# ZhenlongYuan/TSAR-MVS

Hardware: AMD Instinct MI355X
Metric: depthmap Mpixels/sec (ETH3D full-res, 8 iters) (higher is better)
Workload: dtype f32

## Files before the change

### include/tsar.h

```cpp
#ifndef TSAR_H_
#define TSAR_H_

#include <stddef.h>
#include <stdint.h>

#ifdef __cplusplus
extern "C" {
#endif

#define TSAR_MAX_VIEWS 64
#define TSAR_MAXCOST 2.0f

#define TSAR_OK 0
#define TSAR_ERR_INVALID (-1)
#define TSAR_ERR_HIP (-2)
#define TSAR_ERR_STATE (-3)
#define TSAR_ERR_NOMEM (-4)

#define TSAR_MEM_HOST 0
#define TSAR_MEM_DEVICE 1

#define TSAR_COMB_ALL 0
#define TSAR_COMB_BEST_N 1
#define TSAR_COMB_ANGLE 2
// ... 159 lines not shown
void* tsar_device_alloc(int device, size_t bytes);
void tsar_device_free(int device, void* p);
int tsar_device_write(int device, void* dst, const void* host_src, size_t bytes);
int tsar_peer_copy(int dst_device, void* dst, int src_device, const void* src, size_t bytes);

int tsar_enable_kernel_timing(tsar_ctx* ctx, int enable);
int tsar_reset_kernel_timing(tsar_ctx* ctx);
int tsar_get_kernel_timing(tsar_ctx* ctx, tsar_kernel_timing* out, int cap, int* n_out);

int tsar_selftest_sqrt(tsar_ctx* ctx, int mode, uint64_t seed, uint64_t* mismatches_out);
int tsar_selftest_divide(tsar_ctx* ctx, const float* X, const float* Y, const float* Z, size_t n, float* u_out, float* v_out, int ieee);
int tsar_selftest_divide_random(tsar_ctx* ctx, int log2_triples, uint64_t seed, int mode, int guarded, uint64_t* mismatches_out,
                                uint64_t* outside_guard_out);
int tsar_selftest_sweep_census(tsar_ctx* ctx, int colour, uint64_t* out8);
int tsar_selftest_sweep_repeat(tsar_ctx* ctx, int colour, void* memo_dev, uint64_t* out8);
int tsar_selftest_slic_stage(tsar_ctx* ctx, int stage, int w, int h, int mw, int mh, const tsar_slic_settings* s, const void* in0,
                             const void* in1, void* inout);

#ifdef __cplusplus
}
#endif
#endif
```

### tsar-mvs_amd/api.py

```python
from __future__ import annotations

import ctypes as C
import os

import numpy as np

_HERE = os.path.dirname(os.path.abspath(__file__))
LIB_PATH = os.environ.get("TSAR_LIB") or os.path.join(_HERE, "libtsar_hip.so")

TSAR_OK = 0
TSAR_ERR_INVALID, TSAR_ERR_HIP, TSAR_ERR_STATE, TSAR_ERR_NOMEM = -1, -2, -3, -4
MEM_HOST, MEM_DEVICE = 0, 1
COMB_ALL, COMB_BEST_N, COMB_ANGLE, COMB_GOOD = 0, 1, 2, 3
FLAG_FIX_DOWN_FAR_SEED, FLAG_FIX_RIGHT_FAR_CMP, FLAG_STRICT_DIV = 1, 2, 4
FLAG_FIX_PLANE_FIT = 8
FLAG_NO_LINE_CLOSING = 16
FLAG_TEX_FILTER_8BIT = 32
FLAG_FIX_INIT_RADIUS = 64
MAXCOST = 2.0
MAX_VIEWS = 64


class TsarError(RuntimeError):
    def __init__(self, code, msg):
# ... 42 lines not shown
ABI_SYMBOLS = [
    "tsar_create", "tsar_destroy", "tsar_last_error", "tsar_version", "tsar_get_stream", "tsar_synchronize",
    "tsar_default_params", "tsar_set_params", "tsar_set_views", "tsar_set_views_u8", "tsar_set_view_subset",
    "tsar_pm_init", "tsar_pm_iterate", "tsar_pm_iterate_final", "tsar_pm_sweep", "tsar_set_sweep_counter", "tsar_pm_cost_planes", "tsar_set_plane", "tsar_get_plane",
    "tsar_load_planes", "tsar_compute_disp", "tsar_compute_disp_final", "tsar_depth_to_plane", "tsar_get_result",
    "tsar_pyramid_views", "tsar_upsample_planes", "tsar_compute_disp_final_upsampled", "tsar_get_view_image",
    "tsar_set_geom_depths", "tsar_clear_geom", "tsar_pm_rescore", "tsar_get_geom_matrices",
    "tsar_geom_pyramid", "tsar_pyramid_planes", "tsar_upsample_merge",
    "tsar_default_geom_check_params", "tsar_geom_check",
    "tsar_default_geom_reproject_params", "tsar_geom_reproject", "tsar_pm_merge_depths",
    "tsar_default_plane_prior_params", "tsar_set_plane_prior", "tsar_clear_plane_prior", "tsar_get_plane_prior",
    "tsar_set_reliable_mask", "tsar_get_reliable_mask", "tsar_lrdiff", "tsar_getview", "tsar_wmf", "tsar_set_regions", "tsar_detect_weak_texture", "tsar_ransac_regions",
    "tsar_set_region_planes", "tsar_fake_depth", "tsar_fill_textureless",
    "tsar_default_slic_settings", "tsar_slic", "tsar_default_fusion_params", "tsar_fuse", "tsar_fuse_ctx",
    "tsar_host_alloc", "tsar_host_free", "tsar_device_alloc", "tsar_device_free", "tsar_device_write", "tsar_peer_copy", "tsar_enable_kernel_timing", "tsar_reset_kernel_timing", "tsar_get_kernel_timing",
    "tsar_selftest_divide", "tsar_selftest_divide_random", "tsar_selftest_sqrt", "tsar_selftest_sweep_census", "tsar_selftest_sweep_repeat", "tsar_selftest_slic_stage",
]

_lib = None


def load_library(path: str = LIB_PATH):
    global _lib
    if _lib is not None:
        return _lib
    if not os.path.exists(path):
        raise ImportError(f"{path} not found: build it with `make -C tsar-mvs_amd/csrc` "
                          "(or __graft_entry__.build()); there is no CPU fallback")
    L = C.CDLL(path)
    L.tsar_last_error.restype = C.c_char_p
    L.tsar_last_error.argtypes = [C.c_void_p]
# ... 66 lines not shown
    L.tsar_fake_depth.argtypes = [C.c_void_p, C.c_void_p, C.c_int]
    L.tsar_fill_textureless.argtypes = [C.c_void_p]
    L.tsar_slic.argtypes = [C.c_void_p, C.c_void_p, C.c_int, C.c_int, C.POINTER(SlicSettings), C.c_void_p, C.c_int]
    L.tsar_default_fusion_params.restype = None
    L.tsar_default_fusion_params.argtypes = [C.POINTER(FusionParams)]
    L.tsar_fuse.argtypes = [C.c_int, C.c_int, C.c_int, C.c_int, C.POINTER(Camera), C.POINTER(C.c_void_p), C.POINTER(C.c_void_p), C.POINTER(C.c_void_p), C.c_int,
                            C.c_void_p, C.c_void_p, C.POINTER(FusionParams), C.c_void_p, C.c_int64, C.POINTER(C.c_int64)]
    L.tsar_fuse_ctx.argtypes = [C.c_void_p] + list(L.tsar_fuse.argtypes[1:])
    L.tsar_get_stream.argtypes = [C.c_void_p, C.POINTER(C.c_void_p)]
    L.tsar_synchronize.argtypes = [C.c_void_p]
    L.tsar_enable_kernel_timing.argtypes = [C.c_void_p, C.c_int]
    L.tsar_reset_kernel_timing.argtypes = [C.c_void_p]
    L.tsar_get_kernel_timing.argtypes = [C.c_void_p, C.POINTER(KernelTiming), C.c_int, C.POINTER(C.c_int)]
    L.tsar_selftest_divide.argtypes = [C.c_void_p, C.c_void_p, C.c_void_p, C.c_void_p, C.c_size_t, C.c_void_p, C.c_void_p, C.c_int]
    L.tsar_selftest_sweep_census.argtypes = [C.c_void_p, C.c_int, C.POINTER(C.c_uint64)]
    L.tsar_selftest_sweep_repeat.argtypes = [C.c_void_p, C.c_int, C.c_void_p, C.POINTER(C.c_uint64)]
    L.tsar_selftest_sqrt.argtypes = [C.c_void_p, C.c_int, C.c_uint64, C.POINTER(C.c_uint64)]
    L.tsar_selftest_divide_random.argtypes = [C.c_void_p, C.c_int, C.c_uint64, C.c_int, C.c_int, C.POINTER(C.c_uint64), C.POINTER(C.c_uint64)]
    L.tsar_selftest_slic_stage.argtypes = [C.c_void_p, C.c_int, C.c_int, C.c_int, C.c_int, C.c_int, C.POINTER(SlicSettings), C.c_void_p, C.c_void_p, C.c_void_p]
    _lib = L
    return L


def default_params(**kw) -> Params:
    p = Params()
    load_library().tsar_default_params(C.byref(p))
    for k, v in kw.items():
        setattr(p, k, v)
    return p

# ... 305 lines not shown
        assert X.shape == Y.shape == Z.shape
        u, v = np.empty_like(X), np.empty_like(X)
        self._chk(self.L.tsar_selftest_divide(self._ctx, _ptr(X)[0], _ptr(Y)[0], _ptr(Z)[0], X.size, _ptr(u)[0], _ptr(v)[0], int(ieee) if mode is None else mode))
        return u, v

    def selftest_sqrt(self, mode: int, seed: int = 0) -> int:
        bad = C.c_uint64(0)
        self._chk(self.L.tsar_selftest_sqrt(self._ctx, mode, seed, C.byref(bad)))
        return bad.value

    def selftest_sweep_census(self, colour: int) -> dict:
        out = (C.c_uint64 * 8)()
        self._chk(self.L.tsar_selftest_sweep_census(self._ctx, colour, out))
        keys = ("waves", "arms_any_lane", "max_lane_survivors", "max_lane_survivors_nodup", "lane_survivors", "lane_survivors_nodup", "pixels", "arms_present")
        return dict(zip(keys, [int(v) for v in out]))

    def selftest_divide_random(self, log2_triples: int, seed: int, mode: int, guarded: bool = True):
        bad, out = C.c_uint64(0), C.c_uint64(0)
        self._chk(self.L.tsar_selftest_divide_random(self._ctx, log2_triples, seed, mode, int(guarded), C.byref(bad), C.byref(out)))
        return bad.value, out.value

    def _slic_stage(self, stage, w, h, mw, mh, settings, in0, in1, inout):
        p1 = _ptr(in1)[0] if in1 is not None else None
        self._chk(self.L.tsar_selftest_slic_stage(self._ctx, stage, w, h, mw, mh, C.byref(settings), _ptr(in0)[0], p1, _ptr(inout)[0]))
        return inout

    def slic_convert(self, bgra, color_space=0):
        img = np.ascontiguousarray(bgra, np.uint8).reshape(-1, 4)
        return self._slic_stage(0, img.shape[0], 1, 0, 0, SlicSettings(20, 0, 5.0, 0, color_space), img, None, np.zeros((img.shape[0], 4), np.float32))

# ... 272 lines not shown
```

### tsar-mvs_amd/csrc/pm_core.h

```cpp
#pragma once
#include <type_traits>

#include "tsar_device_math.h"

#define PM_BLOCK 256
#define PM_RW 32

#include "pm_tap_common.h"

template <bool QUAD, bool DIFF = false>
DEVFN float sample_bilinear(const DevView& vw, int w, int h, int qpitch, float u, float v, bool q8 = false) {
    u = fminf(fmaxf(u, -1.0f), (float)w);
    v = fminf(fmaxf(v, -1.0f), (float)h);
    const float fu = floorf(u), fv = floorf(v);
    float ax = u - fu, ay = v - fv;
    if (q8) { ax = rintf(ax * 256.0f) * 0.00390625f; ay = rintf(ay * 256.0f) * 0.00390625f; }
    const int iu = (int)fu, iv = (int)fv;
    float t00, t10, t01, t11;
    if (QUAD) {
        const uint32_t off = (uint32_t)(__mul24(iv + 1, qpitch) + iu + 1) * 4u;
        const uint32_t q = *(global_u32_ptr)((const char __attribute__((address_space(1)))*)vw.quad + off);
        t00 = (float)(q & 0xffu);
        t10 = (float)((q >> 8) & 0xffu);
        t01 = (float)((q >> 16) & 0xffu);
// ... 134 lines not shown
    const prior_entry q = ((const __attribute__((address_space(1))) prior_entry*)pp)[y * sc->w + x];
    const float Dp = q.w;
    const float a = fabsf(D - Dp);
    const float rel = a / Dp;
    const float dclip = sc->prior_depth_clip, nclip = sc->prior_normal_clip;
    const float r_d = rel < dclip ? rel / dclip : 1.0f;
    const float s = 1.0f - ((n4.x * q.x + n4.y * q.y) + n4.z * q.z);
    const float s0 = s < 0.0f ? 0.0f : s;
    const float r_n = s < nclip ? s0 / nclip : 1.0f;
    const float t = (sc->prior_weight_depth * r_d) + (sc->prior_weight_normal * r_n);
    return Dp > 0.0f ? c + t : c;
}

template <int NB, int HR, bool STRICT, bool QUAD, int V = 0, int BLK = PM_BLOCK>
DEVFN float multiview_cost(const DevScene* __restrict__ sc, const typename TileOf<QUAD>::type* tile, int tw, int own, const float* wts, const PixelRef& pr,
                           int x, int y, const float4& n4, int& beview, float& ratio) {
    constexpr bool GEOM = (V & TSAR_V_GEOM) != 0;
    constexpr int VT = V & ~(TSAR_V_GEOM | TSAR_V_REDRAW);
    float best[NB];
#pragma unroll
    for (int k = 0; k < NB; k++) best[k] = __builtin_inff();
    const int num = sc->n_sel;
    int valid = 0, bv = -1;
    float cmin = __builtin_inff();
    float depth_h = 0.0f;
    if constexpr (GEOM) depth_h = plane_depth(sc->ref, n4, x, y);
    int vi_next = sc->sel[0];
    for (int i = 0; i < num; i++) {
        const int vi = vi_next;
        vi_next = sc->sel[i + 1 < num ? i + 1 : i];
        float c;
        if constexpr ((VT & TSAR_V_LUT) != 0) c = view_cost_lut<STRICT, (VT >> 11) & 7, (VT & TSAR_V_BUF) != 0 && !STRICT, (VT & TSAR_V_MIX) != 0 && !STRICT>(sc, sc->view[vi], tile, tw, own, wts, pr, x, y, n4);
        else if constexpr (QUAD && HR == 5 && r5_production_variant(VT))
            c = view_cost_r5<STRICT, (VT & 128) != 0 && !STRICT, (VT & 8) != 0, (VT & TSAR_V_BUF) != 0, (VT & TSAR_V_MIX) != 0, BLK>(sc, sc->view[vi], tile, tw, own, wts, pr, x, y, n4);
#ifdef TSAR_EXPERIMENTS
        else if constexpr (QUAD && HR == 5 && r5_diag_variant(VT))
            c = view_cost_r5<false, true, true, true, true, BLK, (VT & 4194304) ? 1 : 2>(sc, sc->view[vi], tile, tw, own, wts, pr, x, y, n4);
#endif
        else {
            static_assert(VT == 0, "unknown tap-loop variant");
            c = view_cost_generic<HR, STRICT, QUAD, BLK>(sc, sc->view[vi], tile, tw, own, wts, pr, x, y, n4);
        }
        auto vmin = [](float a, float b) { float r; asm("v_min_f32 %0, %1, %2" : "=v"(r) : "v"(a), "v"(b)); return r; };
        auto vmax = [](float a, float b) { float r; asm("v_max_f32 %0, %1, %2" : "=v"(r) : "v"(a), "v"(b)); return r; };
        c = vmin(c, TSAR_MAXCOST);
        valid -= (int32_t)__float_as_uint(c - TSAR_MAXCOST) >> 31;
        if constexpr (GEOM) c = c + geom_term(sc, sc->view[vi], vi, x, y, depth_h);
        {
// ... 47 lines not shown
```

### tsar-mvs_amd/csrc/pm_sweep.hip

```cpp
#include "pm_sweep_impl.h"

__global__ void d16_probe_kernel(uint32_t* out) {
    __shared__ unsigned short t[64];
    t[threadIdx.x] = (unsigned short)(0x4300u + threadIdx.x);
    __syncthreads();
    uint32_t r = 0xffffffffu;
    const uint32_t addr = (uint32_t)(uintptr_t)(const __attribute__((address_space(3))) unsigned short*)(t + threadIdx.x);
    asm volatile("ds_read_u16_d16_hi %0, %1\n\ts_waitcnt lgkmcnt(0)" : "+v"(r) : "v"(addr));
    out[threadIdx.x] = r;
}
bool probe_d16_hi_zeroes(tsar_ctx* ctx) {
    CallFrame f(ctx, "d16 probe", nullptr, false);
    uint32_t h[64];
    uint32_t* d = f.out(h, 64, TSAR_MEM_HOST);
    if (f.ok()) {
        hipLaunchKernelGGL(d16_probe_kernel, dim3(1), dim3(64), 0, ctx->stream, d);
        f.launched();
    }
    bool ok = f.finish() == TSAR_OK;
    for (int i = 0; ok && i < 64; i++) ok = h[i] == ((0x4300u + i) << 16);
    return ok;
}

template <int NB, int HR>
static int launch_sweep_nh(tsar_ctx* ctx, int colour, const PlaneBuf& a, const PlaneBuf& b, const PlaneBuf& c, uint32_t sid, int dp, int dr) {
    const bool strict = ctx->hscene.flags & TSAR_FLAG_STRICT_DIV, quad = ctx->hscene.use_quad;
    const bool buf = ctx->buffer_gather && ctx->sweeps_done >= (strict ? (ctx->buffer_from > 2 ? ctx->buffer_from : 2) : ctx->buffer_from);
    const int v = ctx->variant;
    if constexpr ((NB == 2 || NB == 4) && HR == 5)
    if (quad && !(ctx->hscene.flags & TSAR_FLAG_TEX_FILTER_8BIT) && (v == 250 || v == 122 || (v == 114 && NB == 2))) {
#define SWEEP_R5(S, V, B) (buf ? launch_sweep_g<NB, 5, S, true, (V) | TSAR_V_BUF, B>(ctx, colour, a, b, c, sid, dp, dr) : launch_sweep_g<NB, 5, S, true, V, B>(ctx, colour, a, b, c, sid, dp, dr))
        const bool mix = buf && !strict && v == 250 && ctx->hscene.n_sel > 0 && ctx->hscene.view[ctx->hscene.sel[0]].dquad != nullptr;
#define SWEEP_R5_FAST250(B) (mix ? launch_sweep_g<NB, 5, false, true, 250 | TSAR_V_BUF | TSAR_V_MIX, B>(ctx, colour, a, b, c, sid, dp, dr) : SWEEP_R5(false, 250, B))
        if constexpr (NB == 2) {
            const int tiles256 = ((ctx->hscene.w + PM_RW - 1) / PM_RW) * ((ctx->hscene.h + 15) / 16);
            bool small = tiles256 < SWEEP_SMALL_IMAGE_TILES;
            if (ctx->force_block) small = ctx->force_block == 128;
            if (small && v != 114) {
                if (strict) return SWEEP_R5(true, 122, 128);
                return v == 250 ? SWEEP_R5_FAST250(128) : launch_sweep_g<2, 5, false, true, 122, 128>(ctx, colour, a, b, c, sid, dp, dr);
            }
            if (v == 114) return strict ? launch_sweep_g<2, 5, true, true, 114>(ctx, colour, a, b, c, sid, dp, dr) : launch_sweep_g<2, 5, false, true, 114>(ctx, colour, a, b, c, sid, dp, dr);
        }
        if (strict) return SWEEP_R5(true, 122, PM_BLOCK);
        return v == 250 ? SWEEP_R5_FAST250(PM_BLOCK) : launch_sweep_g<NB, 5, false, true, 122>(ctx, colour, a, b, c, sid, dp, dr);
#undef SWEEP_R5_FAST250
#undef SWEEP_R5
    }
    constexpr int NBG = NB == 4 ? 32 : NB;
    if (strict) return quad ? launch_sweep_g<NBG, HR, true, true>(ctx, colour, a, b, c, sid, dp, dr) : launch_sweep_g<NBG, HR, true, false>(ctx, colour, a, b, c, sid, dp, dr);
    return quad ? launch_sweep_g<NBG, HR, false, true>(ctx, colour, a, b, c, sid, dp, dr) : launch_sweep_g<NBG, HR, false, false>(ctx, colour, a, b, c, sid, dp, dr);
}

int launch_pm_sweep(tsar_ctx* ctx, int colour, const PlaneBuf& same_in, const PlaneBuf& other, const PlaneBuf& same_out, uint32_t stream_id,
                    int do_prop, int do_refine) {
    const DevScene& hs = ctx->hscene;
#ifdef TSAR_EXPERIMENTS
    if (!scene_has_terms(hs)) {
        int launched = 0;
        const int rc = launch_pm_sweep_experiment(ctx, colour, same_in, other, same_out, stream_id, do_prop, do_refine, &launched);
        if (rc != TSAR_OK || launched) return rc;
// ... 13 lines not shown
```

### tsar-mvs_amd/csrc/pm_sweep_impl.h

```cpp
#pragma once
#include "pm_dispatch.h"

#define SWEEP_SMALL_IMAGE_TILES 3072

#define CAND_SAME (1 << 30)

DEVFN void select_candidates(const DevScene* __restrict__ sc, const float* __restrict__ c_same, const float* __restrict__ c_other,
                             int x, int y, int cand[8]) {
    const int col = sc->w, row = sc->h;
    const int p = y * col + x;
    const bool fix_seed = sc->flags & TSAR_FLAG_FIX_DOWN_FAR_SEED, fix_cmp = sc->flags & TSAR_FLAG_FIX_RIGHT_FAR_CMP;
    float cmin;
    int cp, cs;
#pragma unroll
    for (int k = 0; k < 8; k++) cand[k] = -1;
    if (y > 2) {
        cp = p - 3 * col; cmin = c_other[cp];
#pragma unroll
        for (int i = 1; i < 11; ++i)
            if (y > 2 + 2 * i) { const int q = p - (3 + 2 * i) * col; const float v = c_other[q]; if (v < cmin) { cmin = v; cp = q; } }
        cand[0] = cp;
    }
    if (y < row - 3) {
        cp = p + 3 * col;
// ... 60 lines not shown
    }
}

DEVFN bool same_bits(const float4& a, const float4& b) {
    return __float_as_uint(a.x) == __float_as_uint(b.x) && __float_as_uint(a.y) == __float_as_uint(b.y) &&
           __float_as_uint(a.z) == __float_as_uint(b.z) && __float_as_uint(a.w) == __float_as_uint(b.w);
}

struct SweepMemo {
    int32_t* cand;
    uint32_t* seq;
    uint32_t* changed;
    uint32_t launch, valid_from;
    int mode;
    int slot_off;
};

template <int NB, int HR, bool STRICT, bool QUAD, int V = 0, int BLK = PM_BLOCK, bool CMP = false>
__global__ __launch_bounds__(BLK) void pm_sweep_kernel(const DevScene* __restrict__ sc, int colour,
                                                            const float* __restrict__ c_same, const float4* __restrict__ n_same,
                                                            const float* __restrict__ c_other, const float4* __restrict__ n_other,
                                                            float* c_out, float4* n_out, float* __restrict__ ratio_out,
                                                            int32_t* __restrict__ beview_out, uint32_t stream_id, int do_prop,
                                                            int do_refine, int tiles_x, int n_tiles, int cost_consistent, int strip_w,
                                                            const float* __restrict__ final_text, SweepMemo memo) {
    extern __shared__ __attribute__((aligned(16))) unsigned char lds_raw[];
    typedef typename TileOf<QUAD>::type TileT;
    constexpr int RW = PM_RW;
    constexpr int SWEEP_RH = 2 * BLK / RW;
    const int hr = HR > 0 ? HR : sc->hrad, vr = HR > 0 ? HR : sc->vrad;
    const int tw = RW + 2 * hr, th = SWEEP_RH + 2 * vr;
// ... 99 lines not shown
                    const float dispOut = fminf(fmaxf(disp + dz, sc->min_disp), sc->max_disp);
                    depth_t = fb / dispOut;
                    float nt[3];
                    nt[0] = n_now.x + between(rn.u[1], -deltaN, deltaN);
                    nt[1] = n_now.y + between(rn.u[2], -deltaN, deltaN);
                    nt[2] = n_now.z + between(rn.u[3], -deltaN, deltaN);
                    const float inv = 1.0f / sqrtf(dot3(nt, nt));
                    nt[0] *= inv; nt[1] *= inv; nt[2] *= inv;
                    if (dot3(nt, vv) > 0.0f) { nt[0] = -nt[0]; nt[1] = -nt[1]; nt[2] = -nt[2]; }
                    n_t.x = nt[0]; n_t.y = nt[1]; n_t.z = nt[2];
                    n_t.w = plane_offset(rf, nt, x, y, depth_t);
                    deltaN = deltaN / 4.0f;
                    deltaZ = deltaZ / 10.0f;
                }
                int bv; float rt;
                const float cost_t = multiview_cost<NB, HR, STRICT, QUAD, V, BLK>(sc, tile, tw, own, wts, pr, x, y, n_t, bv, rt);
                if (cost_t < cost_now) {
                    cost_now = cost_t; n_now = n_t; depth_now = depth_t;
                    ratio_w = rt; beview_w = bv; wrote = true;
                }
            }
        }
    } else {
        const int lane = threadIdx.x & 63, wave0 = threadIdx.x & ~63;
        volatile int32_t* slot_ci = (volatile int32_t*)(lds_raw + memo.slot_off) + wave0;
        volatile unsigned short* slot_src = (volatile unsigned short*)(lds_raw + memo.slot_off + 4 * BLK) + wave0;
        auto pixel_of = [&](int tid, int& px, int& py, int& pown) {
            const int sly = tid >> 4, sk = tid & 15;
            py = ty0 + sly;
            const int slx = 2 * sk + ((colour + py) & 1);
            px = tx0 + slx;
// ... 89 lines not shown
                    depth_t = fb / dispOut;
                    float nt[3];
                    nt[0] = n_now.x + between(rn.u[1], -dN, dN);
                    nt[1] = n_now.y + between(rn.u[2], -dN, dN);
                    nt[2] = n_now.z + between(rn.u[3], -dN, dN);
                    const float inv = 1.0f / sqrtf(dot3(nt, nt));
                    nt[0] *= inv; nt[1] *= inv; nt[2] *= inv;
                    if (dot3(nt, ev) > 0.0f) { nt[0] = -nt[0]; nt[1] = -nt[1]; nt[2] = -nt[2]; }
                    n_t.x = nt[0]; n_t.y = nt[1]; n_t.z = nt[2];
                    n_t.w = plane_offset(rf, nt, ex, ey, depth_t);
                }
            }
            const float* ewts = LUTW ? wts_base : wts_base + etid;
            int bv = -1;
            float rt = 0.f, cost_t = TSAR_MAXCOST;
            if (go) cost_t = multiview_cost<NB, HR, STRICT, QUAD, V, BLK>(sc, tile, tw, eown, ewts, epr, ex, ey, n_t, bv, rt);
            if (it < trips) {
                arms_of_trip(lo, [&](int a, int j, bool has) {
                    const float c = __int_as_float(__builtin_amdgcn_ds_bpermute((j & 63) << 2, __float_as_int(cost_t)));
                    const float r = __int_as_float(__builtin_amdgcn_ds_bpermute((j & 63) << 2, __float_as_int(rt)));
                    const int b = __builtin_amdgcn_ds_bpermute((j & 63) << 2, bv);
                    if (has && c < cost_now) {
                        cost_now = c; acc_arm = a;
                        ratio_w = r; beview_w = b;
                    }
                });
            } else if (go && cost_t < cost_now) {
                cost_now = cost_t; n_now = n_t; depth_now = depth_t;
                ratio_w = rt; beview_w = bv;
            }
        }
// ... 11 lines not shown
            c_out[pp] = cost_now;
            n_out[pp] = n_now;
            if (changed && !final_text) { ratio_out[pp] = ratio_w; beview_out[pp] = beview_w; }
            if (changed && memo.mode) memo.changed[pp] = memo.launch;
            return;
        }
    }
    c_out[p] = cost_now;
    n_out[p] = n_now;
    if (wrote && !final_text) { ratio_out[p] = ratio_w; beview_out[p] = beview_w; }
    if (wrote && memo.mode) memo.changed[p] = memo.launch;
}


template <int HR, bool QUAD, int V>
constexpr bool sweep_has_packed_form() { return QUAD && ((HR == 5 && r5_production_variant(V & ~TSAR_V_GEOM)) || (V & TSAR_V_LUT) != 0); }

template <int NB, int HR, bool STRICT, bool QUAD, int V = 0, int BLK = PM_BLOCK>
static int launch_sweep_t(tsar_ctx* ctx, int colour, const PlaneBuf& same_in, const PlaneBuf& other, const PlaneBuf& same_out,
                          uint32_t stream_id, int do_prop, int do_refine) {
    constexpr int SWEEP_RH = 2 * BLK / PM_RW;
#ifdef TSAR_EXPERIMENTS
    const size_t lds_pad = ctx->lds_pad;
#else
    constexpr size_t lds_pad = 0;
#endif
    SweepMemo memo;
    memo.cand = ctx->memo_cand; memo.seq = ctx->memo_seq; memo.changed = ctx->changed_seq;
    memo.launch = ctx->launch_seq; memo.valid_from = ctx->memo_valid_from;
    memo.mode = (ctx->memo_mode && ctx->memo_cand && ctx->cost_consistent && !ctx->final_text) ? 1 : 0;
    bool packed = false;
    if constexpr (sweep_has_packed_form<HR, QUAD, V>())
        packed = memo.mode && do_prop && ctx->compact_from >= 0 && ctx->call_launch >= ctx->compact_from;
    auto kern = pm_sweep_kernel<NB, HR, STRICT, QUAD, V, BLK, false>;
    if constexpr (sweep_has_packed_form<HR, QUAD, V>())
        if (packed) kern = pm_sweep_kernel<NB, HR, STRICT, QUAD, V, BLK, true>;
    const size_t slots = packed ? 6 * (size_t)BLK : 0;
    TapGrid g;
    if (const int rc = tap_grid(ctx, kern, SWEEP_RH, BLK, QUAD, V, lds_pad + slots, g)) return rc;
    memo.slot_off = packed ? (int)(g.lds - slots) : 0;
    {
        ScopedKernelTimer tm(ctx, (V & TSAR_V_GEOM) ? "pm_sweep_geom" : "pm_sweep");
        ScopedKernelTimer tm_packed(ctx, packed ? "pm_sweep_packed" : nullptr);
        hipLaunchKernelGGL(kern, dim3(g.n_tiles), dim3(BLK), g.lds, ctx->stream, ctx->dscene, colour, same_in.c, same_in.n4, other.c,
                           other.n4, same_out.c, same_out.n4, ctx->ratio, ctx->beview, stream_id, do_prop, do_refine, g.tiles_x, g.n_tiles,
                           ctx->cost_consistent ? 1 : 0, strip_width(ctx->strip_w, g.tiles_x), ctx->final_text, memo);
    }
    TSAR_HIP_TRY(ctx, hipGetLastError());
    return TSAR_OK;
}

template <int NB, int HR, bool STRICT, bool QUAD, int V = 0, int BLK = PM_BLOCK>
static int launch_sweep_g(tsar_ctx* ctx, int colour, const PlaneBuf& same_in, const PlaneBuf& other, const PlaneBuf& same_out,
                          uint32_t stream_id, int do_prop, int do_refine) {
    if (scene_has_terms(ctx->hscene)) return launch_sweep_t<NB, HR, STRICT, QUAD, V | TSAR_V_GEOM, BLK>(ctx, colour, same_in, other, same_out, stream_id, do_prop, do_refine);
    return launch_sweep_t<NB, HR, STRICT, QUAD, V, BLK>(ctx, colour, same_in, other, same_out, stream_id, do_prop, do_refine);
}
```

### tsar-mvs_amd/csrc/pm_tap_common.h

```cpp
#pragma once

typedef const uint32_t __attribute__((address_space(1)))* global_u32_ptr;
typedef const float __attribute__((address_space(1)))* global_f32_ptr;

template <bool STRICT, bool ROW = false>
DEVFN void tap_line_base(const float* H, float a, float& bx, float& by, float& bz) {
    bx = STRICT ? H[0] * a : fma_(H[ROW ? 1 : 0], a, H[2]);
    by = STRICT ? H[3] * a : fma_(H[ROW ? 4 : 3], a, H[5]);
    bz = STRICT ? H[6] * a : fma_(H[ROW ? 7 : 6], a, H[8]);
}
template <bool STRICT, bool ROW = false>
DEVFN void tap_homogeneous(const float* H, float t, float bx, float by, float bz, float& X, float& Y, float& Z) {
    X = fma_(H[ROW ? 0 : 1], t, bx); Y = fma_(H[ROW ? 3 : 4], t, by); Z = fma_(H[ROW ? 6 : 7], t, bz);
    if (STRICT) { X += H[2]; Y += H[5]; Z += H[8]; }
}
DEVFN void pixel_homogeneous(const float* H, float xi, float yj, float& X, float& Y, float& Z) {
    float bx, by, bz;
    tap_line_base<false>(H, xi, bx, by, bz);
    tap_homogeneous<false>(H, yj, bx, by, bz, X, Y, Z);
}

template <bool STRICT, bool GUARD>
DEVFN void tap_divide(float X, float Y, float Z, float& u, float& v) {
    if (STRICT) {
// ... 99 lines not shown
    float mean_ref;
    float var_ref;
    bool textured;
};
DEVFN PixelRef pixel_ref_from_sums(float sum_ref, float sum_ref_ref, float inv_wsum) {
    PixelRef pr;
    pr.inv_wsum = inv_wsum;
    sum_ref *= pr.inv_wsum;
    sum_ref_ref *= pr.inv_wsum;
    pr.mean_ref = sum_ref;
    pr.var_ref = sum_ref_ref - sum_ref * sum_ref;
    pr.textured = !(pr.var_ref < 1e-5f);
    return pr;
}

DEVFN float ncc_cost(const PixelRef& pr, TapSums t) {
    t.src *= pr.inv_wsum;
    t.src_src *= pr.inv_wsum;
    t.ref_src *= pr.inv_wsum;
    const float var_src = t.src_src - t.src * t.src;
    if (var_src < 1e-5f) return TSAR_MAXCOST;
    const float covar = t.ref_src - pr.mean_ref * t.src;
    const float vrs = sqrt_rsq_exact(pr.var_ref * var_src);
    return fmaxf(0.0f, fminf(TSAR_MAXCOST, 1.0f - covar / vrs));
}
```

### tsar-mvs_amd/csrc/pm_tap_r5.h

```cpp
#pragma once

template <bool STRICT, bool ROW, bool D16, bool BUF, bool MIX, int BLK, int DIAG = 0>
DEVFN float view_cost_r5(const DevScene* __restrict__ sc, const DevView& vw, const unsigned short* tile, int tw, int own, const float* wts,
                         const PixelRef& pr, int x, int y, const float4& n4) {
    static_assert(!(STRICT && ROW), "the row-wise walk changes the summation order: fast mode only");
    static_assert(!MIX || (BUF && !STRICT), "the half-float difference texture serves the fast arithmetic's blend through buffer loads");
    const int w = sc->w, h = sc->h, qp = sc->quad_pitch;
    const int qorg = quad_border_bytes(qp);
    float H[9];
    if (STRICT) plane_homography(sc->ref, vw, n4, H, sc->k_sparse != 0);
    else plane_homography_fast(sc->ref, vw, n4, H);
    float sum_src = 0.f, sum_src_src = 0.f, sum_ref_src = 0.f;
    bool need_clamp;
    if (!STRICT) {
        float Xc, Yc, Zc;
        pixel_homogeneous(H, (float)x, (float)y, Xc, Yc, Zc);
        const float a = fabsf(H[0]) + fabsf(H[1]), b = fabsf(H[3]) + fabsf(H[4]), c = fabsf(H[6]) + fabsf(H[7]);
        const float Zmin = fma_(-5.0f, c, Zc);
        const float r = __builtin_amdgcn_rcpf(Zmin * Zc);
        const float r5 = 5.0f * r, rc = Zmin * r;
        const float du = fma_(a, Zc, fabsf(Xc) * c) * r5, dv = fma_(b, Zc, fabsf(Yc) * c) * r5;
        const float uc = Xc * rc, vc = Yc * rc;
        const bool inside = Zmin > 0.0f && fminf(uc - du, vc - dv) >= 1.5f && uc + du <= (float)(w - 1) - 1.5f && vc + dv <= (float)(h - 1) - 1.5f;
        need_clamp = !__all(inside);
// ... 100 lines not shown
            if (MIX) s = blend_dquad(q2[jj], ax[jj], ay[jj]);
            else s = blend_quad<!STRICT>(q[jj], ax[jj], ay[jj]);
            if (jj == 0 && DIAG != 2) {
                if (D16)
                    asm("s_waitcnt lgkmcnt(0)" : "+v"(rcol[0]), "+v"(rcol[1]), "+v"(rcol[2]), "+v"(rcol[3]), "+v"(rcol[4]), "+v"(rcol[5]),
                        "+v"(wcol[0]), "+v"(wcol[1]), "+v"(wcol[2]), "+v"(s));
                else
                    asm("s_waitcnt lgkmcnt(0)" : "+v"(wcol[0]), "+v"(wcol[1]), "+v"(wcol[2]), "+v"(s));
            }
            const float r = D16 ? rcol[jj] : tile_value(ROW ? tile[own + i * tw + (2 * jj - 5)] : tile[own + (2 * jj - 5) * tw + i]);
            const float wt = wcol[jj >> 1][jj & 1];
            const TapSums t = tap_accumulate<STRICT>(TapSums{sum_src, sum_src_src, sum_ref_src}, wt, r, s);
            sum_src = t.src; sum_src_src = t.src_src; sum_ref_src = t.ref_src;
        }
    };
    if (need_clamp) {
#pragma unroll 1
        for (int i = -5; i <= 5; i += 2) line6(i, std::true_type(), std::false_type());
    } else if constexpr (MIX) {
#pragma unroll
        for (int i = -5; i <= 5; i += 2) line6(i, std::false_type(), std::true_type());
    } else {
#pragma unroll 1
        for (int i = -5; i <= 5; i += 2) line6(i, std::false_type(), std::false_type());
    }
    return ncc_cost(pr, TapSums{sum_src, sum_src_src, sum_ref_src});
}

__host__ __device__ constexpr bool r5_diag_variant(int V) { return V == (250 | TSAR_V_BUF | TSAR_V_MIX | 4194304) || V == (250 | TSAR_V_BUF | TSAR_V_MIX | 8388608); }
__host__ __device__ constexpr bool r5_production_variant(int V) { return V == 114 || V == 122 || V == 250 || V == (114 | TSAR_V_BUF) || V == (122 | TSAR_V_BUF) || V == (250 | TSAR_V_BUF) || V == (250 | TSAR_V_BUF | TSAR_V_MIX); }
```

### tsar-mvs_amd/csrc/tsar_api.hip

```cpp
#include <math.h>
#include <stdio.h>
#include <stdlib.h>
#include <string.h>

#include <algorithm>

#include "tsar_dev.h"

ScopedKernelTimer::ScopedKernelTimer(tsar_ctx* c, const char* name) : ctx(c) {
    if (!ctx->timing || !name) return;
    for (size_t k = 0; k < ctx->timers.size(); k++)
        if (ctx->timers[k].name == name) ti = (int)k;
    if (ti < 0) {
        ctx->timers.emplace_back();
        ctx->timers.back().name = name;
        ti = (int)ctx->timers.size() - 1;
    }
    if (hipEventCreate(&e0) != hipSuccess) { ti = -1; return; }
    if (hipEventCreate(&e1) != hipSuccess) { hipEventDestroy(e0); ti = -1; return; }
    hipEventRecord(e0, ctx->stream);
}
ScopedKernelTimer::~ScopedKernelTimer() {
    if (ti < 0) return;
    hipEventRecord(e1, ctx->stream);
// ... 162 lines not shown
    return "tsar-mvs_amd 0.2.0 (gfx950)";
#endif
}

static void read_knobs(tsar_ctx* ctx) {
    auto num = [](const char* name, int dflt) { const char* e = getenv(name); return e && e[0] ? atoi(e) : dflt; };
    auto on = [](const char* name, bool dflt) { const char* e = getenv(name); return e && e[0] ? e[0] != '0' : dflt; };
    ctx->variant = num("TSAR_VARIANT", ctx->variant);
    ctx->buffer_gather = on("TSAR_BUFFER_GATHER", true);
    ctx->mix_gather = on("TSAR_MIX_GATHER", true);
    ctx->strip_w = num("TSAR_STRIP", -1);
    ctx->buffer_from = num("TSAR_BUFFER_FROM", 1);
    ctx->force_block = num("TSAR_BLOCK", 0);
    ctx->memo_mode = num("TSAR_MEMO", 1);
    ctx->compact_from = num("TSAR_COMPACT_FROM", 6);
    ctx->lut_mode = num("TSAR_LUT", 1);
    ctx->ransac_wgs = num("TSAR_RANSAC_WGS", 8);
    ctx->ransac_chain = num("TSAR_RANSAC_CHAIN", 8);
    ctx->ransac_lookahead = num("TSAR_RANSAC_LOOKAHEAD", 0);
    ctx->ransac_poll_limit = num("TSAR_RANSAC_POLL_LIMIT", 1 << 15);
    ctx->ransac_cooperative = on("TSAR_RANSAC_COOPERATIVE", true);
    ctx->ransac_force_fallback = on("TSAR_RANSAC_FORCE_FALLBACK", false);
    ctx->trace_host = getenv("TSAR_TRACE_HOST") != nullptr;
#ifdef TSAR_EXPERIMENTS
    ctx->lds_pad = (size_t)num("TSAR_LDS_PAD", 0);
#endif
}

extern "C" int tsar_create(int device, tsar_ctx** out) {
    if (!out) return TSAR_ERR_INVALID;
// ... 24 lines not shown
static void free_geom(tsar_ctx* ctx) {
    for (auto& p : ctx->geom_maps) dev_free(p);
    ctx->geom_maps.clear();
    for (auto& p : ctx->hscene.geom_depth) p = nullptr;
    ctx->hscene.geom_on = 0;
}
static void free_prior(tsar_ctx* ctx) {
    dev_free(ctx->prior);
    ctx->hscene.prior = nullptr;
}
static void free_planes(tsar_ctx* ctx) {
    for (int b = 0; b < 2; b++) { dev_free(ctx->buf[b].c); dev_free(ctx->buf[b].n4); }
    dev_free(ctx->ratio); dev_free(ctx->depth); dev_free(ctx->scale); dev_free(ctx->lrdiff); dev_free(ctx->confid);
    dev_free(ctx->fakedepth); dev_free(ctx->beview); dev_free(ctx->canny); dev_free(ctx->out4);
    dev_free(ctx->memo_cand); dev_free(ctx->memo_seq); dev_free(ctx->changed_seq);
    dev_free(ctx->resize4);
    ctx->have_resize = false;
}

extern "C" int tsar_destroy(tsar_ctx* ctx) {
    if (!ctx) return TSAR_OK;
    (void)enter_ctx(ctx);
    if (ctx->stream) hipStreamSynchronize(ctx->stream);
    drain_timers(ctx);
    free_views(ctx);
    free_planes(ctx);
    free_geom(ctx);
    free_prior(ctx);
    dev_free(ctx->dscene); dev_free(ctx->region_text); dev_free(ctx->region_size); dev_free(ctx->region_n4);
    if (ctx->scratch.base) hipFree(ctx->scratch.base);
// ... 985 lines not shown
int launch_sweep_repeat(tsar_ctx* ctx, int colour, unsigned long long* memo, unsigned long long* dout);
extern "C" int tsar_selftest_sweep_repeat(tsar_ctx* ctx, int colour, void* memo_dev, uint64_t* out8) {
    CHECK_CTX(ctx);
    if (!memo_dev || !out8) return fail(ctx, TSAR_ERR_INVALID, "memo_dev / out8 is NULL");
    NEED_VIEWS(ctx);
    NEED_STATE(ctx);
    return run_counters(ctx, 8, out8, [&](unsigned long long* dc) { return launch_sweep_repeat(ctx, colour & 1, (unsigned long long*)memo_dev, dc); });
}
extern "C" int tsar_selftest_sweep_census(tsar_ctx* ctx, int colour, uint64_t* out8) {
    CHECK_CTX(ctx);
    NEED_VIEWS(ctx);
    NEED_STATE(ctx);
    if (!out8) return fail(ctx, TSAR_ERR_INVALID, "out8 is NULL");
    return run_counters(ctx, 8, out8, [&](unsigned long long* dc) { return launch_sweep_census(ctx, colour & 1, dc); });
}
```

### tsar-mvs_amd/csrc/tsar_dev.h

```cpp
#pragma once
#include <hip/hip_runtime.h>
#include <stdint.h>
#include <stdio.h>
#include <stdlib.h>

#include <chrono>
#include <string>
#include <vector>

#include "../../include/tsar.h"

#define TSAR_LUT_LINES 32
#define TSAR_LUT_TAPS 40
#define TSAR_LUT_MAX_CLASSES 144
#define TSAR_MAX_SELECTED 32

struct DevView {
    float K[9];
    float R[9];
    float t[3];
    float t_abs_lo;
    float A[9];
    float b[3];
    float t_abs_hi;
// ... 35 lines not shown
    int lut_d2[TSAR_LUT_MAX_CLASSES];
    uint32_t tap_row[TSAR_LUT_LINES * TSAR_LUT_TAPS + 8];
    const float* geom_depth[TSAR_MAX_VIEWS];
    float geom_back[TSAR_MAX_VIEWS][12];
    float geom_weight, geom_clip, geom_clip_sq;
    int geom_on;
    const float4* prior;
    float prior_weight_depth, prior_weight_normal, prior_depth_clip, prior_normal_clip;
};
static inline bool scene_has_terms(const DevScene& s) { return s.geom_on != 0 || s.prior != nullptr; }

#define TSAR_V_LUT 1024
#define TSAR_V_BUF 131072
#define TSAR_V_MIX 2097152
#define TSAR_V_GEOM 16777216
#define TSAR_V_REDRAW 33554432

struct PlaneBuf {
    float* c;
    float4* n4;
};

struct KernelTimer {
    std::string name;
    int launches = 0;
    float total_ms = 0.f;
    std::vector<std::pair<hipEvent_t, hipEvent_t>> pending;
};

struct ScratchArena {
// ... 22 lines not shown
    bool cost_consistent = false;
    int n_regions = 0;
    float *region_text = nullptr, *region_size = nullptr;
    float4* region_n4 = nullptr;
    int exact_sqrt_probe = 0;
    int exact_div_probe = 0;
    int sweeps_done = 0;
    int32_t* memo_cand = nullptr;
    uint32_t* memo_seq = nullptr;
    uint32_t* changed_seq = nullptr;
    uint32_t launch_seq = 0;
    uint32_t memo_valid_from = 1;
    int call_launch = 0;
    int memo_mode = 1;
    int compact_from = 6;
    std::vector<tsar_camera> cams;
    bool views_u8 = false;
    float4* resize4 = nullptr;
    bool have_resize = false;
    const float* final_text = nullptr;
    std::vector<float*> geom_maps;
    float4* prior = nullptr;
    int variant = 2;
    bool mix_gather = true;
    bool buffer_gather = true;
    int strip_w = -1;
    int buffer_from = 1;
    int force_block = 0;
    int lut_mode = 1;
    int ransac_wgs = 8;
// ... 241 lines not shown
```

Before: 46.98.

## Prune refinement view costs early with a partial-window NCC bound

Adds a pruning variant of the radius-5 row-wise NCC cost. After a few window rows it bounds the best achievable NCC and, when every lane in the wavefront proves the view cannot beat the current cost, skips the rest of that view. It applies only to the first refinement steps, in best-1 photometric mode without geometric or prior terms. If a skipped view leaves a lane whose cost would have improved, the whole multiview cost is recomputed without pruning, to keep results exact. The cost is an extra partial reference-sum loop per row, loss of the MIX unrolled path while pruning, extra template instantiations, and an optional atomic census for diagnostics.

```diff
diff --git a/include/tsar.h b/include/tsar.h
--- a/include/tsar.h
+++ b/include/tsar.h
@@ -197,6 +197,7 @@
                                 uint64_t* outside_guard_out);
 int tsar_selftest_sweep_census(tsar_ctx* ctx, int colour, uint64_t* out8);
 int tsar_selftest_sweep_repeat(tsar_ctx* ctx, int colour, void* memo_dev, uint64_t* out8);
+int tsar_selftest_prune_census(tsar_ctx* ctx, int on, uint32_t* out32);
 int tsar_selftest_slic_stage(tsar_ctx* ctx, int stage, int w, int h, int mw, int mh, const tsar_slic_settings* s, const void* in0,
                              const void* in1, void* inout);
 
diff --git a/tsar-mvs_amd/api.py b/tsar-mvs_amd/api.py
--- a/tsar-mvs_amd/api.py
+++ b/tsar-mvs_amd/api.py
@@ -80,7 +80,7 @@
     "tsar_set_region_planes", "tsar_fake_depth", "tsar_fill_textureless",
     "tsar_default_slic_settings", "tsar_slic", "tsar_default_fusion_params", "tsar_fuse", "tsar_fuse_ctx",
     "tsar_host_alloc", "tsar_host_free", "tsar_device_alloc", "tsar_device_free", "tsar_device_write", "tsar_peer_copy", "tsar_enable_kernel_timing", "tsar_reset_kernel_timing", "tsar_get_kernel_timing",
-    "tsar_selftest_divide", "tsar_selftest_divide_random", "tsar_selftest_sqrt", "tsar_selftest_sweep_census", "tsar_selftest_sweep_repeat", "tsar_selftest_slic_stage",
+    "tsar_selftest_divide", "tsar_selftest_divide_random", "tsar_selftest_sqrt", "tsar_selftest_sweep_census", "tsar_selftest_prune_census", "tsar_selftest_sweep_repeat", "tsar_selftest_slic_stage",
 ]
 
 _lib = None
@@ -177,6 +177,8 @@
     L.tsar_get_kernel_timing.argtypes = [C.c_void_p, C.POINTER(KernelTiming), C.c_int, C.POINTER(C.c_int)]
     L.tsar_selftest_divide.argtypes = [C.c_void_p, C.c_void_p, C.c_void_p, C.c_void_p, C.c_size_t, C.c_void_p, C.c_void_p, C.c_int]
     L.tsar_selftest_sweep_census.argtypes = [C.c_void_p, C.c_int, C.POINTER(C.c_uint64)]
+    if hasattr(L, "tsar_selftest_prune_census"):
+        L.tsar_selftest_prune_census.argtypes = [C.c_void_p, C.c_int, C.POINTER(C.c_uint32)]
     L.tsar_selftest_sweep_repeat.argtypes = [C.c_void_p, C.c_int, C.c_void_p, C.POINTER(C.c_uint64)]
     L.tsar_selftest_sqrt.argtypes = [C.c_void_p, C.c_int, C.c_uint64, C.POINTER(C.c_uint64)]
     L.tsar_selftest_divide_random.argtypes = [C.c_void_p, C.c_int, C.c_uint64, C.c_int, C.c_int, C.POINTER(C.c_uint64), C.POINTER(C.c_uint64)]
@@ -512,6 +514,14 @@
         self._chk(self.L.tsar_selftest_sweep_census(self._ctx, colour, out))
         keys = ("waves", "arms_any_lane", "max_lane_survivors", "max_lane_survivors_nodup", "lane_survivors", "lane_survivors_nodup", "pixels", "arms_present")
         return dict(zip(keys, [int(v) for v in out]))
+
+    def selftest_prune_census(self, on: bool):
+        if on:
+            self._chk(self.L.tsar_selftest_prune_census(self._ctx, 1, None))
+            return None
+        out = (C.c_uint32 * 32)()
+        self._chk(self.L.tsar_selftest_prune_census(self._ctx, 0, out))
+        return np.array(out, np.int64).reshape(8, 4)
 
     def selftest_divide_random(self, log2_triples: int, seed: int, mode: int, guarded: bool = True):
         bad, out = C.c_uint64(0), C.c_uint64(0)
diff --git a/tsar-mvs_amd/csrc/pm_core.h b/tsar-mvs_amd/csrc/pm_core.h
--- a/tsar-mvs_amd/csrc/pm_core.h
+++ b/tsar-mvs_amd/csrc/pm_core.h
@@ -172,9 +172,11 @@
 
 template <int NB, int HR, bool STRICT, bool QUAD, int V = 0, int BLK = PM_BLOCK>
 DEVFN float multiview_cost(const DevScene* __restrict__ sc, const typename TileOf<QUAD>::type* tile, int tw, int own, const float* wts, const PixelRef& pr,
-                           int x, int y, const float4& n4, int& beview, float& ratio) {
+                           int x, int y, const float4& n4, int& beview, float& ratio, bool prune = false, float cost_now = 0.0f, int* skipped = nullptr) {
     constexpr bool GEOM = (V & TSAR_V_GEOM) != 0;
-    constexpr int VT = V & ~(TSAR_V_GEOM | TSAR_V_REDRAW);
+    constexpr bool PRUNE = (V & TSAR_V_PRUNE) != 0;
+    static_assert(!PRUNE || !GEOM, "the bound speaks of the photometric cost alone");
+    constexpr int VT = V & ~(TSAR_V_GEOM | TSAR_V_REDRAW | TSAR_V_PRUNE);
     float best[NB];
 #pragma unroll
     for (int k = 0; k < NB; k++) best[k] = __builtin_inff();
@@ -189,7 +191,14 @@
         vi_next = sc->sel[i + 1 < num ? i + 1 : i];
         float c;
         if constexpr ((VT & TSAR_V_LUT) != 0) c = view_cost_lut<STRICT, (VT >> 11) & 7, (VT & TSAR_V_BUF) != 0 && !STRICT, (VT & TSAR_V_MIX) != 0 && !STRICT>(sc, sc->view[vi], tile, tw, own, wts, pr, x, y, n4);
-        else if constexpr (QUAD && HR == 5 && r5_production_variant(VT))
+        else if constexpr (QUAD && HR == 5 && r5_production_variant(VT) && PRUNE) {
+            static_assert((VT & 250) == 250 && !STRICT, "pruning instantiations exist for the fast row-wise loop");
+            ViewPrune vp;
+            vp.on = prune; vp.skipped = false;
+            vp.cost_now = cmin < cost_now ? TSAR_MAXCOST : cost_now;
+            c = view_cost_r5<false, true, true, (VT & TSAR_V_BUF) != 0, (VT & TSAR_V_MIX) != 0, BLK, 0, true>(sc, sc->view[vi], tile, tw, own, wts, pr, x, y, n4, &vp);
+            if (vp.skipped) *skipped += 1;
+        } else if constexpr (QUAD && HR == 5 && r5_production_variant(VT))
             c = view_cost_r5<STRICT, (VT & 128) != 0 && !STRICT, (VT & 8) != 0, (VT & TSAR_V_BUF) != 0, (VT & TSAR_V_MIX) != 0, BLK>(sc, sc->view[vi], tile, tw, own, wts, pr, x, y, n4);
 #ifdef TSAR_EXPERIMENTS
         else if constexpr (QUAD && HR == 5 && r5_diag_variant(VT))
diff --git a/tsar-mvs_amd/csrc/pm_sweep.hip b/tsar-mvs_amd/csrc/pm_sweep.hip
--- a/tsar-mvs_amd/csrc/pm_sweep.hip
+++ b/tsar-mvs_amd/csrc/pm_sweep.hip
@@ -31,7 +31,13 @@
     if (quad && !(ctx->hscene.flags & TSAR_FLAG_TEX_FILTER_8BIT) && (v == 250 || v == 122 || (v == 114 && NB == 2))) {
 #define SWEEP_R5(S, V, B) (buf ? launch_sweep_g<NB, 5, S, true, (V) | TSAR_V_BUF, B>(ctx, colour, a, b, c, sid, dp, dr) : launch_sweep_g<NB, 5, S, true, V, B>(ctx, colour, a, b, c, sid, dp, dr))
         const bool mix = buf && !strict && v == 250 && ctx->hscene.n_sel > 0 && ctx->hscene.view[ctx->hscene.sel[0]].dquad != nullptr;
-#define SWEEP_R5_FAST250(B) (mix ? launch_sweep_g<NB, 5, false, true, 250 | TSAR_V_BUF | TSAR_V_MIX, B>(ctx, colour, a, b, c, sid, dp, dr) : SWEEP_R5(false, 250, B))
+#define SWEEP_R5_FAST250_ALL(B) (mix ? launch_sweep_g<NB, 5, false, true, 250 | TSAR_V_BUF | TSAR_V_MIX, B>(ctx, colour, a, b, c, sid, dp, dr) : SWEEP_R5(false, 250, B))
+        const bool prune = NB == 2 && !strict && v == 250 && ctx->prune && ctx->prune_steps > 0 && dr && ctx->call_launch >= ctx->prune_from &&
+                           ctx->hscene.cost_comb == TSAR_COMB_BEST_N && ctx->hscene.n_best == 1 && !scene_has_terms(ctx->hscene);
+#define SWEEP_R5_PRUNE(B) (mix ? launch_sweep_t<2, 5, false, true, 250 | TSAR_V_BUF | TSAR_V_MIX | TSAR_V_PRUNE, B>(ctx, colour, a, b, c, sid, dp, dr) \
+                           : buf ? launch_sweep_t<2, 5, false, true, 250 | TSAR_V_BUF | TSAR_V_PRUNE, B>(ctx, colour, a, b, c, sid, dp, dr)              \
+                                 : launch_sweep_t<2, 5, false, true, 250 | TSAR_V_PRUNE, B>(ctx, colour, a, b, c, sid, dp, dr))
+#define SWEEP_R5_FAST250(B) (prune ? SWEEP_R5_PRUNE(B) : SWEEP_R5_FAST250_ALL(B))
         if constexpr (NB == 2) {
             const int tiles256 = ((ctx->hscene.w + PM_RW - 1) / PM_RW) * ((ctx->hscene.h + 15) / 16);
             bool small = tiles256 < SWEEP_SMALL_IMAGE_TILES;
@@ -45,6 +51,8 @@
         if (strict) return SWEEP_R5(true, 122, PM_BLOCK);
         return v == 250 ? SWEEP_R5_FAST250(PM_BLOCK) : launch_sweep_g<NB, 5, false, true, 122>(ctx, colour, a, b, c, sid, dp, dr);
 #undef SWEEP_R5_FAST250
+#undef SWEEP_R5_PRUNE
+#undef SWEEP_R5_FAST250_ALL
 #undef SWEEP_R5
     }
     constexpr int NBG = NB == 4 ? 32 : NB;
diff --git a/tsar-mvs_amd/csrc/pm_sweep_impl.h b/tsar-mvs_amd/csrc/pm_sweep_impl.h
--- a/tsar-mvs_amd/csrc/pm_sweep_impl.h
+++ b/tsar-mvs_amd/csrc/pm_sweep_impl.h
@@ -98,7 +98,36 @@
     uint32_t launch, valid_from;
     int mode;
     int slot_off;
+    int prune_steps;
+    uint32_t* prune_counts;
 };
+
+template <int NB, int HR, bool STRICT, bool QUAD, int V, int BLK>
+DEVFN float pruned_cost(const DevScene* __restrict__ sc, const typename TileOf<QUAD>::type* tile, int tw, int own, const float* wts, const PixelRef& pr,
+                        int x, int y, const float4& n4, int& beview, float& ratio, int step, float cost_now, int prune_steps, uint32_t* prune_counts) {
+    if constexpr ((V & TSAR_V_PRUNE) == 0) {
+        return multiview_cost<NB, HR, STRICT, QUAD, V, BLK>(sc, tile, tw, own, wts, pr, x, y, n4, beview, ratio);
+    } else {
+        bool prune = step >= 0 && step < prune_steps;
+        float c;
+#pragma unroll 1
+        for (;;) {
+            int skipped = 0;
+            c = multiview_cost<NB, HR, STRICT, QUAD, V, BLK>(sc, tile, tw, own, wts, pr, x, y, n4, beview, ratio, prune, cost_now, &skipped);
+            const bool redo = skipped != 0 && __any(c < cost_now);
+            if (prune && prune_counts != nullptr) {
+                const uint64_t act = __ballot(1);
+                if ((threadIdx.x & 63) == __ffsll((long long)act) - 1) {
+                    uint32_t* k = prune_counts + 4 * step;
+                    atomicAdd(k + 0, 1u); atomicAdd(k + 1, (uint32_t)sc->n_sel); atomicAdd(k + 2, (uint32_t)skipped); atomicAdd(k + 3, redo ? 1u : 0u);
+                }
+            }
+            if (!redo) break;
+            prune = false;
+        }
+        return c;
+    }
+}
 
 template <int NB, int HR, bool STRICT, bool QUAD, int V = 0, int BLK = PM_BLOCK, bool CMP = false>
 __global__ __launch_bounds__(BLK) void pm_sweep_kernel(const DevScene* __restrict__ sc, int colour,
@@ -228,7 +257,7 @@
                     deltaZ = deltaZ / 10.0f;
                 }
                 int bv; float rt;
-                const float cost_t = multiview_cost<NB, HR, STRICT, QUAD, V, BLK>(sc, tile, tw, own, wts, pr, x, y, n_t, bv, rt);
+                const float cost_t = pruned_cost<NB, HR, STRICT, QUAD, V, BLK>(sc, tile, tw, own, wts, pr, x, y, n_t, bv, rt, h - 8, cost_now, memo.prune_steps, memo.prune_counts);
                 if (cost_t < cost_now) {
                     cost_now = cost_t; n_now = n_t; depth_now = depth_t;
                     ratio_w = rt; beview_w = bv; wrote = true;
@@ -348,7 +377,7 @@
             const float* ewts = LUTW ? wts_base : wts_base + etid;
             int bv = -1;
             float rt = 0.f, cost_t = TSAR_MAXCOST;
-            if (go) cost_t = multiview_cost<NB, HR, STRICT, QUAD, V, BLK>(sc, tile, tw, eown, ewts, epr, ex, ey, n_t, bv, rt);
+            if (go) cost_t = pruned_cost<NB, HR, STRICT, QUAD, V, BLK>(sc, tile, tw, eown, ewts, epr, ex, ey, n_t, bv, rt, it - trips, cost_now, memo.prune_steps, memo.prune_counts);
             if (it < trips) {
                 arms_of_trip(lo, [&](int a, int j, bool has) {
                     const float c = __int_as_float(__builtin_amdgcn_ds_bpermute((j & 63) << 2, __float_as_int(cost_t)));
@@ -390,7 +419,7 @@
 
 
 template <int HR, bool QUAD, int V>
-constexpr bool sweep_has_packed_form() { return QUAD && ((HR == 5 && r5_production_variant(V & ~TSAR_V_GEOM)) || (V & TSAR_V_LUT) != 0); }
+constexpr bool sweep_has_packed_form() { return QUAD && ((HR == 5 && r5_production_variant(V & ~(TSAR_V_GEOM | TSAR_V_PRUNE))) || (V & TSAR_V_LUT) != 0); }
 
 template <int NB, int HR, bool STRICT, bool QUAD, int V = 0, int BLK = PM_BLOCK>
 static int launch_sweep_t(tsar_ctx* ctx, int colour, const PlaneBuf& same_in, const PlaneBuf& other, const PlaneBuf& same_out,
@@ -405,6 +434,8 @@
     memo.cand = ctx->memo_cand; memo.seq = ctx->memo_seq; memo.changed = ctx->changed_seq;
     memo.launch = ctx->launch_seq; memo.valid_from = ctx->memo_valid_from;
     memo.mode = (ctx->memo_mode && ctx->memo_cand && ctx->cost_consistent && !ctx->final_text) ? 1 : 0;
+    memo.prune_steps = ((V & TSAR_V_PRUNE) != 0 && do_refine && ctx->call_launch >= ctx->prune_from) ? ctx->prune_steps : 0;
+    memo.prune_counts = (V & TSAR_V_PRUNE) != 0 ? ctx->prune_counts : nullptr;
     bool packed = false;
     if constexpr (sweep_has_packed_form<HR, QUAD, V>())
         packed = memo.mode && do_prop && ctx->compact_from >= 0 && ctx->call_launch >= ctx->compact_from;
@@ -418,6 +449,7 @@
     {
         ScopedKernelTimer tm(ctx, (V & TSAR_V_GEOM) ? "pm_sweep_geom" : "pm_sweep");
         ScopedKernelTimer tm_packed(ctx, packed ? "pm_sweep_packed" : nullptr);
+        ScopedKernelTimer tm_prune(ctx, (V & TSAR_V_PRUNE) ? "pm_sweep_prune" : nullptr);
         hipLaunchKernelGGL(kern, dim3(g.n_tiles), dim3(BLK), g.lds, ctx->stream, ctx->dscene, colour, same_in.c, same_in.n4, other.c,
                            other.n4, same_out.c, same_out.n4, ctx->ratio, ctx->beview, stream_id, do_prop, do_refine, g.tiles_x, g.n_tiles,
                            ctx->cost_consistent ? 1 : 0, strip_width(ctx->strip_w, g.tiles_x), ctx->final_text, memo);
diff --git a/tsar-mvs_amd/csrc/pm_tap_common.h b/tsar-mvs_amd/csrc/pm_tap_common.h
--- a/tsar-mvs_amd/csrc/pm_tap_common.h
+++ b/tsar-mvs_amd/csrc/pm_tap_common.h
@@ -137,6 +137,30 @@
     return pr;
 }
 
+struct ViewPrune {
+    float cost_now;
+    bool on;
+    bool skipped;
+};
+#define PM_PRUNE_E 0.9f
+#define PM_PRUNE_EA 0.45f
+#define PM_PRUNE_SLACK 1.0e-4f
+DEVFN bool prune_proven(const TapSums& t, float aw, float ar, float arr, const PixelRef& pr, float cost_now) {
+    const float E = PM_PRUNE_EA * aw * aw;
+    const float a_lo = fma_(aw, arr, -(ar * ar)) - E;
+    const float b_lo = fma_(aw, t.src_src, -(t.src * t.src)) - E;
+    const float c_hi = fabsf(fma_(aw, t.ref_src, -(ar * t.src))) + E;
+    const float raw = __builtin_amdgcn_rcpf(aw);
+    const float q = fma_(-(c_hi * c_hi), __builtin_amdgcn_rcpf(b_lo), a_lo) * raw;
+    const float vs = (b_lo * raw) * pr.inv_wsum, vr = pr.var_ref - PM_PRUNE_E;
+    const float n2 = fma_(-q, pr.inv_wsum * __builtin_amdgcn_rcpf(pr.var_ref + PM_PRUNE_E), 1.0f);
+    const float eg = PM_PRUNE_E * __builtin_amdgcn_rsqf(vr * vs);
+    const float tt = 1.0f - cost_now;
+    const float lhs = fma_(eg, 2.0f + eg, n2);
+    const float rhs = (fma_(tt, tt, -PM_PRUNE_SLACK) * (1.0f - PM_PRUNE_E * __builtin_amdgcn_rcpf(vr))) * (1.0f - PM_PRUNE_E * __builtin_amdgcn_rcpf(vs));
+    return cost_now < 1.0f && vr >= 2.0f * PM_PRUNE_E && vs >= 2.0f * PM_PRUNE_E && lhs <= rhs;
+}
+
 DEVFN float ncc_cost(const PixelRef& pr, TapSums t) {
     t.src *= pr.inv_wsum;
     t.src_src *= pr.inv_wsum;
diff --git a/tsar-mvs_amd/csrc/pm_tap_r5.h b/tsar-mvs_amd/csrc/pm_tap_r5.h
--- a/tsar-mvs_amd/csrc/pm_tap_r5.h
+++ b/tsar-mvs_amd/csrc/pm_tap_r5.h
@@ -1,9 +1,13 @@
 #pragma once
 
-template <bool STRICT, bool ROW, bool D16, bool BUF, bool MIX, int BLK, int DIAG = 0>
+#define PM_PRUNE_FIRST_LINE 2
+#define PM_PRUNE_LAST_LINE 4
+
+template <bool STRICT, bool ROW, bool D16, bool BUF, bool MIX, int BLK, int DIAG = 0, bool PRUNE = false>
 DEVFN float view_cost_r5(const DevScene* __restrict__ sc, const DevView& vw, const unsigned short* tile, int tw, int own, const float* wts,
-                         const PixelRef& pr, int x, int y, const float4& n4) {
+                         const PixelRef& pr, int x, int y, const float4& n4, ViewPrune* vp = nullptr) {
     static_assert(!(STRICT && ROW), "the row-wise walk changes the summation order: fast mode only");
+    static_assert(!PRUNE || (ROW && D16 && !STRICT && DIAG == 0), "the partial-window bound is written for the fast row-wise loop");
     static_assert(!MIX || (BUF && !STRICT), "the half-float difference texture serves the fast arithmetic's blend through buffer loads");
     const int w = sc->w, h = sc->h, qp = sc->quad_pitch;
     const int qorg = quad_border_bytes(qp);
@@ -138,15 +142,35 @@
             sum_src = t.src; sum_src_src = t.src_src; sum_ref_src = t.ref_src;
         }
     };
+    auto pruned = [&](int line) {
+        if constexpr (PRUNE) {
+            if (vp->on && line >= PM_PRUNE_FIRST_LINE - 1 && line < PM_PRUNE_LAST_LINE) {
+                float pa_w = 0.f, pa_r = 0.f, pa_rr = 0.f;
+#pragma unroll 1
+                for (int l = 0; l <= line; l++) {
+#pragma unroll
+                    for (int jj = 0; jj < 6; jj++) {
+                        const float wt = wts[(6 * jj + l) * BLK], r = tile_value(tile[own + (2 * l - 5) * tw + (2 * jj - 5)]);
+                        const float wr = wt * r;
+                        pa_w += wt;
+                        pa_r += wr;
+                        pa_rr = fma_(wr, r, pa_rr);
+                    }
+                }
+                if (__all(prune_proven(TapSums{sum_src, sum_src_src, sum_ref_src}, pa_w, pa_r, pa_rr, pr, vp->cost_now))) { vp->skipped = true; return true; }
+            }
+        }
+        return false;
+    };
     if (need_clamp) {
 #pragma unroll 1
-        for (int i = -5; i <= 5; i += 2) line6(i, std::true_type(), std::false_type());
-    } else if constexpr (MIX) {
+        for (int i = -5; i <= 5; i += 2) { line6(i, std::true_type(), std::false_type()); if (pruned((i + 5) >> 1)) return TSAR_MAXCOST; }
+    } else if (MIX && !(PRUNE && vp->on)) {
 #pragma unroll
-        for (int i = -5; i <= 5; i += 2) line6(i, std::false_type(), std::true_type());
+        for (int i = -5; i <= 5; i += 2) line6(i, std::false_type(), std::bool_constant<MIX>());
     } else {
 #pragma unroll 1
-        for (int i = -5; i <= 5; i += 2) line6(i, std::false_type(), std::false_type());
+        for (int i = -5; i <= 5; i += 2) { line6(i, std::false_type(), std::false_type()); if (pruned((i + 5) >> 1)) return TSAR_MAXCOST; }
     }
     return ncc_cost(pr, TapSums{sum_src, sum_src_src, sum_ref_src});
 }
diff --git a/tsar-mvs_amd/csrc/tsar_api.hip b/tsar-mvs_amd/csrc/tsar_api.hip
--- a/tsar-mvs_amd/csrc/tsar_api.hip
+++ b/tsar-mvs_amd/csrc/tsar_api.hip
@@ -200,6 +200,9 @@
     ctx->force_block = num("TSAR_BLOCK", 0);
     ctx->memo_mode = num("TSAR_MEMO", 1);
     ctx->compact_from = num("TSAR_COMPACT_FROM", 6);
+    ctx->prune = num("TSAR_PRUNE", 1);
+    ctx->prune_steps = std::min(std::max(num("TSAR_PRUNE_STEPS", 2), 0), 8);
+    ctx->prune_from = num("TSAR_PRUNE_FROM", 1);
     ctx->lut_mode = num("TSAR_LUT", 1);
     ctx->ransac_wgs = num("TSAR_RANSAC_WGS", 8);
     ctx->ransac_chain = num("TSAR_RANSAC_CHAIN", 8);
@@ -254,6 +257,7 @@
     dev_free(ctx->ratio); dev_free(ctx->depth); dev_free(ctx->scale); dev_free(ctx->lrdiff); dev_free(ctx->confid);
     dev_free(ctx->fakedepth); dev_free(ctx->beview); dev_free(ctx->canny); dev_free(ctx->out4);
     dev_free(ctx->memo_cand); dev_free(ctx->memo_seq); dev_free(ctx->changed_seq);
+    if (ctx->prune_counts) { (void)hipFree(ctx->prune_counts); ctx->prune_counts = nullptr; }
     dev_free(ctx->resize4);
     ctx->have_resize = false;
 }
@@ -1269,3 +1273,17 @@
     if (!out8) return fail(ctx, TSAR_ERR_INVALID, "out8 is NULL");
     return run_counters(ctx, 8, out8, [&](unsigned long long* dc) { return launch_sweep_census(ctx, colour & 1, dc); });
 }
+extern "C" int tsar_selftest_prune_census(tsar_ctx* ctx, int on, uint32_t* out32) {
+    CHECK_CTX(ctx);
+    TSAR_HIP_TRY(ctx, hipStreamSynchronize(ctx->stream));
+    if (on) {
+        if (!ctx->prune_counts) TSAR_HIP_TRY(ctx, hipMalloc((void**)&ctx->prune_counts, 32 * sizeof(uint32_t)));
+        TSAR_HIP_TRY(ctx, hipMemset(ctx->prune_counts, 0, 32 * sizeof(uint32_t)));
+        return TSAR_OK;
+    }
+    if (!ctx->prune_counts) return fail(ctx, TSAR_ERR_INVALID, "no prune census is running");
+    if (out32) TSAR_HIP_TRY(ctx, hipMemcpy(out32, ctx->prune_counts, 32 * sizeof(uint32_t), hipMemcpyDeviceToHost));
+    TSAR_HIP_TRY(ctx, hipFree(ctx->prune_counts));
+    ctx->prune_counts = nullptr;
+    return TSAR_OK;
+}
diff --git a/tsar-mvs_amd/csrc/tsar_dev.h b/tsar-mvs_amd/csrc/tsar_dev.h
--- a/tsar-mvs_amd/csrc/tsar_dev.h
+++ b/tsar-mvs_amd/csrc/tsar_dev.h
@@ -73,6 +73,7 @@
 #define TSAR_V_BUF 131072
 #define TSAR_V_MIX 2097152
 #define TSAR_V_GEOM 16777216
+#define TSAR_V_PRUNE 67108864
 #define TSAR_V_REDRAW 33554432
 
 struct PlaneBuf {
@@ -125,6 +126,10 @@
     int call_launch = 0;
     int memo_mode = 1;
     int compact_from = 6;
+    int prune = 1;
+    int prune_steps = 2;
+    int prune_from = 1;
+    uint32_t* prune_counts = nullptr;
     std::vector<tsar_camera> cams;
     bool views_u8 = false;
     float4* resize4 = nullptr;
```

Measured after the change: 49.15, median of 6. 4.6% higher.
